# rust-cv/cv

Measured on NVIDIA H100. Metric: vSLAM frames/s (AKAZE+match+RANSAC, 1080p ~5k kp) at 1/2/4/8 H100, higher is better.
Workload: dtype f32+f64

## Files before the change

### cv_b200/csrc/arrsac_dev.cuh

```cuda
#pragma once

#define ARS_SORT_CAP 4096u
#define ARS_BOOK_NT 1024
#define ARS_BOOK_SMEM (14u * ARS_SORT_CAP)
#define ARS_QCAP (1u << 20)

struct ArrsacCtl {
    uint32_t n, init_n, Mv, npass;
    uint32_t Hn, cur, blk_lo, blk_hi;
    uint32_t acc_hi, n_new, worst, done;
    uint32_t found, iters, nraw, q_count;
    uint32_t q_count2, stat_lazy;
    uint32_t stat_units0, stat_units2;
    uint32_t stat_repairs, stat_pad;
    uint64_t rng_pos, gen_pos;
    cvb_rng gen;
    cvb_pose winner;
    uint32_t n_inliers, overflow;
    uint32_t stat_chunks, stat_pass;
    uint32_t stat_walk_us, stat_commit_us;
    uint32_t stat_perm_us, stat_turns;
};

struct ArrsacParams {
    uint32_t K, MM, kind;
    uint32_t H0, ib, bs, max_cand, G;
    uint32_t W0;
    uint32_t NW;
    uint32_t NMAX;
    uint32_t rows;
    uint32_t prefix, cmin;
    float lr_thr, eps0, delta0;
    double thr;
    int row0;
};

__device__ __forceinline__ unsigned long long ars_globaltimer() { unsigned long long t; asm volatile("mov.u64 %0, %%globaltimer;" : "=l"(t)); return t; }
__device__ __forceinline__ uint64_t ars_rotl64(uint64_t x, int k) { return (x << k) | (x >> (64 - k)); }
__device__ uint32_t ars_rng_next_u32(cvb_rng *r) {
    if (r->kind == 0) {
        uint64_t *s = r->s;
        const uint64_t result = ars_rotl64(s[0] + s[3], 23) + s[0];
        const uint64_t t = s[1] << 17;
        s[2] ^= s[0]; s[3] ^= s[1]; s[1] ^= s[2]; s[0] ^= s[3]; s[2] ^= t; s[3] = ars_rotl64(s[3], 45);
        return (uint32_t)(result >> 32);
    }
    unsigned __int128 state = (unsigned __int128)r->s[0] | ((unsigned __int128)r->s[1] << 64);
    const unsigned __int128 incr = (unsigned __int128)r->s[2] | ((unsigned __int128)r->s[3] << 64);
    const unsigned __int128 MUL = ((unsigned __int128)0x2360ED051FC65DA4ull << 64) | 0x4385DF649FCCF645ull;
    state = state * MUL + incr;
    r->s[0] = (uint64_t)state; r->s[1] = (uint64_t)(state >> 64);
    const uint32_t rot = (uint32_t)(state >> 122);
    const uint64_t xsl = (uint64_t)(state >> 64) ^ (uint64_t)state;
    return (uint32_t)((xsl >> rot) | (xsl << ((64 - rot) & 63)));
// ... 103 lines not shown
            }
            while (c < K) {
                const uint32_t s = ars_raw_at(ctl, raw, pos) % len;
                pos++;
                bool dup = false;
                for (uint32_t j = 0; j < c; j++) dup |= loc[j] == s;
                if (!dup) loc[c++] = s;
            }
            for (uint32_t k = 0; k < K; k++) out[(size_t)(h0 + f) * K + k] = loc[k];
            sh[0] = h0 + f + 1; *(uint64_t *)(sh + 2) = pos;
        } else if (f >= m && tid == 0) {
            sh[0] = h0 + m; *(uint64_t *)(sh + 2) = p0 + (uint64_t)m * K;
        }
        __syncthreads();
    }
    const uint32_t hdone = sh[0];
    __syncthreads();
    if (tid == 0) ctl->rng_pos = *(const uint64_t *)(sh + 2);
    __syncthreads();
    if (hdone < count) ars_sample_block(ctl, raw, len, K, count - hdone, out + (size_t)hdone * K, nullptr, win, sh);
}

__global__ void __launch_bounds__(ARS_BOOK_NT) k_ars_begin(ArrsacCtl *ctl, ArrsacParams P, const uint32_t *n_dev, uint32_t n_host,
                                                            const uint32_t *raw, uint32_t *samples0) {
    __shared__ uint32_t win[ARS_WIN];
    __shared__ __align__(8) uint32_t sh[4];
    const uint32_t n = min(n_dev ? *n_dev : n_host, P.NMAX);
    if (threadIdx.x == 0) {
        ctl->n = n;
        ctl->init_n = min(P.bs * P.ib, n);
        ctl->Mv = 0; ctl->npass = 0; ctl->Hn = 0; ctl->cur = 0; ctl->blk_lo = ctl->blk_hi = ctl->acc_hi = 0;
        ctl->n_new = 0; ctl->worst = 0; ctl->found = 0; ctl->iters = 0; ctl->n_inliers = 0; ctl->overflow = 0;
        ctl->stat_chunks = 0; ctl->stat_pass = 0; ctl->q_count = 0; ctl->q_count2 = 0; ctl->stat_lazy = 0; ctl->stat_units0 = 0; ctl->stat_units2 = 0; ctl->stat_repairs = 0; ctl->stat_pad = 0; ctl->stat_walk_us = 0; ctl->stat_commit_us = 0; ctl->stat_perm_us = 0; ctl->stat_turns = 0;
        ctl->done = (n < P.K || P.H0 == 0) ? 1u : 0u;
    }
    __syncthreads();
    if (n < P.K || P.H0 == 0) return;
    ars_sample_block_par(ctl, raw, n, P.K, P.H0, samples0, win, sh);
}

template <int KIND>
__global__ void __launch_bounds__(128) k_ars_estimate(const ArrsacCtl *ctl, int phase, uint32_t H_init, const double *__restrict__ a,
                                                      const double *__restrict__ b, const uint32_t *__restrict__ samples,
                                                      cvb_pose *poses, uint8_t *nposes, int row0) {
    if (ctl->done) return;
    const uint32_t H = phase == 0 ? H_init : ctl->n_new;
    const uint32_t h = blockIdx.x * blockDim.x + threadIdx.x;
    if (h >= H) return;
    if (KIND == 2) { nposes[h] = (uint8_t)five_point(a, b, samples + (size_t)h * 5, row0, poses + (size_t)h * 40); return; }
    cvb_pose out[4];
    const int n = KIND == 0 ? eight_point(a, b, samples + (size_t)h * 8, out) : p3p(a, b, samples + (size_t)h * 3, out);
    for (int k = 0; k < n; k++) poses[(size_t)h * 4 + k] = out[k];
    nposes[h] = (uint8_t)n;
}

template <int EIGHT_LANES, int MINB>
__global__ void __launch_bounds__(128, MINB) k_ars_estimate8(const ArrsacCtl *ctl, int phase, uint32_t H_init, const double *__restrict__ a,
                                                       const double *__restrict__ b, const uint32_t *__restrict__ samples,
                                                       cvb_pose *poses, uint8_t *nposes) {
    if (ctl->done) return;
    __shared__ double sh[(128 / EIGHT_LANES) * EIGHT_SH];
    const uint32_t H = phase == 0 ? H_init : ctl->n_new;
    const uint32_t g = threadIdx.x / EIGHT_LANES, lane = threadIdx.x % EIGHT_LANES;
    const uint32_t h = blockIdx.x * (128 / EIGHT_LANES) + g;
    if (h >= H) return;
    const unsigned mask = ((1u << EIGHT_LANES) - 1u) << ((threadIdx.x & 31) / EIGHT_LANES * EIGHT_LANES);
    cvb_pose out[4];
    const int n = eight_point_lanes<EIGHT_LANES>(a, b, samples + (size_t)h * 8, out, sh + g * EIGHT_SH, lane, mask);
    if (lane == 0) {
        for (int k = 0; k < n; k++) poses[(size_t)h * 4 + k] = out[k];
        nposes[h] = (uint8_t)n;
    }
}

__device__ __noinline__ bool ars_exact_c2c(const cvb_pose *Pz, const double *pa, const double *pb, double thr) {
    return residual_c2c(*Pz, pa, pb) < thr;
}

template <int RES>
__device__ __forceinline__ bool ars_inlier(const cvb_pose &Pz, const double *__restrict__ a, const double *__restrict__ b, uint32_t i,
                                           double thr) {
    if (RES == 1) return residual_w2c(Pz, a + 3 * (size_t)i, b + 4 * (size_t)i) < thr;
    const double *pa = a + 3 * (size_t)i, *pb = b + 3 * (size_t)i;
    int f = c2c_inlier_filter(Pz.r, Pz.t, pa, pb, thr);
    if (f < 0) f = ars_exact_c2c(&Pz, pa, pb, thr) ? 1 : 0;
    return f != 0;
}

__device__ __forceinline__ bool ars_ready(uint32_t word0, uint32_t init_n, uint32_t sample, const ArrsacParams &P) {
    if (sample < P.prefix) return true;
    const uint32_t c = min(32u, init_n);
    return (uint32_t)__popc(c < 32 ? (word0 & ((1u << c) - 1)) : word0) >= P.cmin;
}

template <int RES>
__global__ void __launch_bounds__(256, 2) k_ars_score(ArrsacCtl *ctl, uint2 *__restrict__ queue, ArrsacParams P, int phase, const double *__restrict__ a,
                                                   const double *__restrict__ b, const cvb_pose *__restrict__ poses0,
                                                   const uint8_t *__restrict__ nposes0, uint32_t *__restrict__ masks0,
                                                   const cvb_pose *__restrict__ tposes, uint32_t *__restrict__ tmasks,
                                                   const cvb_pose *__restrict__ newposes, const uint8_t *__restrict__ nposes_new,
                                                   uint32_t *__restrict__ newmask) {
    if (ctl->done) return;
    const unsigned full = 0xffffffffu;
    const uint32_t lane = threadIdx.x & 31;
    const uint32_t warp = (blockIdx.x * blockDim.x + threadIdx.x) >> 5, nwarps = (gridDim.x * blockDim.x) >> 5;
    if (phase == 0 || phase == 2) {
        const uint32_t init_n = ctl->init_n, W = (init_n + 31) >> 5;
        const uint32_t nmod = P.H0 * P.MM, npre = min(P.prefix, P.H0) * P.MM, W1 = W > 0 ? W - 1 : 0;
        const uint32_t units = phase == 0 ? nmod + npre * W1 : (nmod - npre) * W1;
        uint32_t *qc = phase == 0 ? &ctl->q_count : &ctl->q_count2;
        uint2 *q = phase == 0 ? queue : queue + ARS_QCAP;
        for (uint32_t u = warp; u < units; u += nwarps) {
            uint32_t m, w;
            if (phase == 0) { if (u < nmod) { m = u; w = 0; } else { m = (u - nmod) / W1; w = 1 + (u - nmod) % W1; } }
            else { m = npre + u / W1; w = 1 + u % W1; }
            if ((m % P.MM) >= nposes0[m / P.MM]) continue;
            if (phase == 2 && !ars_ready(masks0[(size_t)m * P.W0], init_n, m / P.MM, P)) continue;
            const uint32_t i = w * 32 + lane;
            bool bit = false;
            if (i < init_n) {
                if (RES == 1) bit = ars_inlier<RES>(poses0[m], a, b, i, P.thr);
                else {
                    const cvb_pose &Pz = poses0[m];
                    const int f = c2c_inlier_filter(Pz.r, Pz.t, a + 3 * (size_t)i, b + 3 * (size_t)i, P.thr);
                    if (f >= 0) bit = f != 0;
                    else {
                        const uint32_t slot = atomicAdd(qc, 1u);
                        if (slot < ARS_QCAP) q[slot] = make_uint2(m, i);
                        else bit = ars_exact_c2c(&Pz, a + 3 * (size_t)i, b + 3 * (size_t)i, P.thr);
                    }
                }
            }
            const unsigned bits = __ballot_sync(full, bit);
            if (lane == 0) { masks0[(size_t)m * P.W0 + w] = bits; atomicAdd(phase == 0 ? &ctl->stat_units0 : &ctl->stat_units2, 1u); }
        }
        return;
    }
    const uint32_t lo = ctl->blk_lo, hi = ctl->blk_hi, Hn = ctl->Hn, cur = ctl->cur;
    const uint32_t wlo = lo >> 5, nwb = hi > lo ? ((hi - 1) >> 5) - wlo + 1 : 0;
    const uint32_t kept_units = Hn * nwb;
    const uint32_t nnew = ctl->n_new * P.MM, nwn = (hi + 31) >> 5;
    const uint32_t units = kept_units + nnew * nwn;
    const cvb_pose *tp = tposes + (size_t)cur * P.rows;
    uint32_t *tm = tmasks + (size_t)cur * P.rows * P.NW;
    for (uint32_t u = warp; u < units; u += nwarps) {
        if (u < kept_units) {
            const uint32_t r = u / nwb, w = wlo + u % nwb;
            const uint32_t i = w * 32 + lane;
            const bool act = i >= lo && i < hi;
            bool bit = false;
            if (act) bit = ars_inlier<RES>(tp[r], a, b, i, P.thr);
            const unsigned bits = __ballot_sync(full, bit), range = __ballot_sync(full, act);
            if (lane == 0) { uint32_t *p = tm + (size_t)r * P.NW + w; *p = (*p & ~range) | bits; }
        } else {
            const uint32_t v = u - kept_units;
            const uint32_t j = v / nwn, w = v % nwn;
            if ((j % P.MM) >= nposes_new[j / P.MM]) continue;
            const uint32_t i = w * 32 + lane;
            bool bit = false;
            if (i < hi) bit = ars_inlier<RES>(newposes[j], a, b, i, P.thr);
            const unsigned bits = __ballot_sync(full, bit);
            if (lane == 0) newmask[(size_t)j * P.NW + w] = bits;
        }
    }
}

__global__ void __launch_bounds__(256) k_ars_resolve(const ArrsacCtl *ctl, const uint2 *__restrict__ queue, int stage, ArrsacParams P,
                                                     const double *__restrict__ a, const double *__restrict__ b,
                                                     const cvb_pose *__restrict__ poses0, uint32_t *__restrict__ masks0) {
    if (ctl->done) return;
    const uint32_t cnt = min(stage == 0 ? ctl->q_count : ctl->q_count2, ARS_QCAP);
    queue += stage == 0 ? 0 : ARS_QCAP;
    for (uint32_t e = blockIdx.x * blockDim.x + threadIdx.x; e < cnt; e += gridDim.x * blockDim.x) {
        const uint2 q = queue[e];
        if (residual_c2c(poses0[q.x], a + 3 * (size_t)q.y, b + 3 * (size_t)q.y) < P.thr)
            atomicOr(&masks0[(size_t)q.x * P.W0 + (q.y >> 5)], 1u << (q.y & 31));
    }
}

__device__ void ars_scan3(uint32_t &a, uint32_t &b, uint32_t &c, uint32_t *sm , uint32_t *tot ) {
    const unsigned full = 0xffffffffu;
    const uint32_t lane = threadIdx.x & 31, wid = threadIdx.x >> 5;
    for (int o = 1; o < 32; o <<= 1) {
        const uint32_t x = __shfl_up_sync(full, a, o), y = __shfl_up_sync(full, b, o), z = __shfl_up_sync(full, c, o);
        if ((int)lane >= o) { a += x; b += y; c += z; }
    }
    __syncthreads();
    if (lane == 31) { sm[wid] = a; sm[32 + wid] = b; sm[64 + wid] = c; }
    __syncthreads();
    if (wid == 0) {
        uint32_t x = sm[lane], y = sm[32 + lane], z = sm[64 + lane];
        for (int o = 1; o < 32; o <<= 1) {
            const uint32_t p = __shfl_up_sync(full, x, o), q = __shfl_up_sync(full, y, o), r = __shfl_up_sync(full, z, o);
            if ((int)lane >= o) { x += p; y += q; z += r; }
        }
        sm[lane] = x; sm[32 + lane] = y; sm[64 + lane] = z;
        if (lane == 31) { tot[0] = x; tot[1] = y; tot[2] = z; }
    }
    __syncthreads();
    if (wid > 0) { a += sm[wid - 1]; b += sm[32 + wid - 1]; c += sm[64 + wid - 1]; }
}

__device__ uint32_t ars_block_min(uint32_t v, uint32_t *sm ) {
    const unsigned full = 0xffffffffu;
    for (int o = 16; o; o >>= 1) v = min(v, __shfl_xor_sync(full, v, o));
    __syncthreads();
    if ((threadIdx.x & 31) == 0) sm[threadIdx.x >> 5] = v;
    __syncthreads();
    uint32_t r = sm[threadIdx.x & 31];
// ... 355 lines not shown
        const uint32_t id = vm[p];
        const double *src = (const double *)(poses0 + id);
        double *dst = (double *)(tposes + r);
        if (lane < 12) dst[lane] = src[lane];
        if (lane == 0) tinl[r] = 0xfffffu - (uint32_t)(kx >> 32);
        for (uint32_t w = lane; w < P.NW; w += 32) tmasks[(size_t)r * P.NW + w] = w < P.W0 ? masks0[(size_t)id * P.W0 + w] : 0u;
    }
    __syncthreads();
    if (tid == 0) {
        const uint32_t n = ctl->n;
        ctl->Hn = Hn; ctl->cur = 0; ctl->stat_pass = npass;
        ctl->acc_hi = init_n; ctl->blk_lo = init_n; ctl->blk_hi = min(init_n + P.bs, n);
        ctl->n_new = 0; ctl->worst = 0;
        if (!(init_n < n && Hn > 1)) {
            ctl->done = 1; ctl->found = Hn >= 1 ? 1 : 0;
            if (Hn >= 1) ctl->winner = tposes[0];
        }
    }
}

__global__ void __launch_bounds__(ARS_BOOK_NT) k_ars_book(ArrsacCtl *ctl, ArrsacParams P, const uint32_t *__restrict__ raw,
                                                           cvb_pose *tposes, uint32_t *tinl, uint32_t *tmasks,
                                                           const cvb_pose *__restrict__ newposes, const uint8_t *__restrict__ nposes_new,
                                                           const uint32_t *__restrict__ newmask, uint32_t *__restrict__ pool,
                                                           uint32_t *__restrict__ samples_new, unsigned long long loop_cond) {
    if (ctl->done) { if (loop_cond && threadIdx.x == 0) cudaGraphSetConditional(loop_cond, 0); return; }
    __shared__ __align__(8) uint32_t sm[96];
    __shared__ uint32_t tot[3];
    extern __shared__ __align__(16) unsigned char ars_dyn[];
    uint64_t *keys = (uint64_t *)ars_dyn;
    uint32_t *e_inl = (uint32_t *)(ars_dyn + 8 * ARS_SORT_CAP);
    uint16_t *e_src = (uint16_t *)(ars_dyn + 12 * ARS_SORT_CAP);
    const uint32_t tid = threadIdx.x, NT = blockDim.x;
    const uint32_t cur = ctl->cur, Hk = ctl->Hn, n = ctl->n;
    const uint32_t acc_hi = ctl->acc_hi, lo = ctl->blk_lo, hi = ctl->blk_hi, worst = ctl->worst;
    const uint32_t nnew = ctl->n_new * P.MM;
    const cvb_pose *tp = tposes + (size_t)cur * P.rows;
    const uint32_t *ti = tinl + (size_t)cur * P.rows;
    const uint32_t *tm = tmasks + (size_t)cur * P.rows * P.NW;
    for (uint32_t r = tid; r < Hk; r += NT) { e_inl[r] = ti[r]; e_src[r] = (uint16_t)r; keys[r] = ars_key(ti[r], r, r); }
    uint32_t total = Hk;
    for (uint32_t j0 = 0; j0 < nnew; j0 += NT) {
        const uint32_t j = j0 + tid;
        uint32_t inl = 0;
        bool acc = false;
        if (j < nnew && (j % P.MM) < nposes_new[j / P.MM]) {
            inl = ars_popc_range(newmask + (size_t)j * P.NW, 0, acc_hi);
            acc = inl > worst;
        }
        uint32_t x = acc ? 1 : 0, y = 0, z = 0;
        ars_scan3(x, y, z, sm, tot);
        if (acc) {
            const uint32_t p = total + x - 1;
            if (p < ARS_SORT_CAP) { e_inl[p] = inl; e_src[p] = (uint16_t)(P.rows + j); keys[p] = ars_key(inl, p, p); }
        }
        total += tot[0];
        __syncthreads();
    }
    uint32_t P2 = ars_pow2(max(total, 2u));
    for (uint32_t i = total + tid; i < P2; i += NT) keys[i] = ~0ull;
    ars_bitonic(keys, P2);
    const uint32_t Hn1 = min(total, P.max_cand);
    if (!(lo < n && Hn1 > 1)) {
        if (tid == 0) {
            ctl->done = 1; ctl->found = Hn1 >= 1 ? 1 : 0;
            if (Hn1 >= 1) {
// ... 100 lines not shown
```

### cv_b200/csrc/c2c_filter.cuh

```cuda
#pragma once
#include <math.h>

#if defined(__CUDACC__)
#define C2C_HD __host__ __device__ __forceinline__
#else
#define C2C_HD static inline
#endif
#if defined(__CUDA_ARCH__)
#define C2C_FMA(a, b, c) fma((a), (b), (c))
#define C2C_RSQRT(a) rsqrt(a)
#else
#define C2C_FMA(a, b, c) ((a) * (b) + (c))
#define C2C_RSQRT(a) (1.0 / sqrt(a))
#endif

C2C_HD int c2c_ldl4(const double *m, double s, double *d, double *l, double *inv) {
    const double tiny = 1e-11;
    const double m00 = m[0] - s, m11 = m[5] - s, m22 = m[10] - s, m33 = m[15] - s;
    const double m10 = m[4], m20 = m[8], m30 = m[12], m21 = m[9], m31 = m[13], m32 = m[14];
    int neg = 0;
    d[0] = m00;
    if (!(fabs(d[0]) > tiny)) return -1;
    neg += d[0] < 0.0;
    const double i0 = 1.0 / d[0];
// ... 48 lines not shown
        const double c0 = C2C_FMA(t[1], ra2, -(t[2] * ra1)), c1 = C2C_FMA(t[2], ra0, -(t[0] * ra2)), c2 = C2C_FMA(t[0], ra1, -(t[1] * ra0));
        const double e = C2C_FMA(b[2], c2, C2C_FMA(b[1], c1, b[0] * c0));
        if (e * e > 8.5 * (tt - 1.0) * thr + 1e-28) return 0;
        if (thr <= 1e-4) {
            const double tb = C2C_FMA(t[2], b[2], C2C_FMA(t[1], b[1], t[0] * b[0])), ub = C2C_FMA(ra2, b[2], C2C_FMA(ra1, b[1], ra0 * b[0])),
                         tu = C2C_FMA(t[2], ra2, C2C_FMA(t[1], ra1, t[0] * ra0));
            const double c1 = C2C_FMA(-ub, tu, tb), c2 = C2C_FMA(ub, tb, -tu);
            const double lim2 = 100.0 * (tt - 1.0) * thr;
            if ((c1 < 0.0 && c1 * c1 > lim2) || (c2 < 0.0 && c2 * c2 > lim2)) return 0;
        }
    }
    double D[16];
    {
        double Ta[3][3];
        for (int c = 0; c < 3; c++)
            for (int r = 0; r < 3; r++) Ta[r][c] = C2C_FMA(-a[r], a[c], r == c ? 1.0 : 0.0);
        double Tb[3][4];
        for (int c = 0; c < 4; c++) {
            const double m0 = c < 3 ? R[c] : t[0], m1 = c < 3 ? R[3 + c] : t[1], m2 = c < 3 ? R[6 + c] : t[2];
            const double btm = C2C_FMA(b[2], m2, C2C_FMA(b[1], m1, b[0] * m0));
            Tb[0][c] = C2C_FMA(-b[0], btm, m0); Tb[1][c] = C2C_FMA(-b[1], btm, m1); Tb[2][c] = C2C_FMA(-b[2], btm, m2);
        }
        for (int i = 0; i < 4; i++)
            for (int j = 0; j <= i; j++) {
                double v = C2C_FMA(Tb[2][i], Tb[2][j], C2C_FMA(Tb[1][i], Tb[1][j], Tb[0][i] * Tb[0][j]));
                if (i < 3) v = C2C_FMA(Ta[2][i], Ta[2][j], C2C_FMA(Ta[1][i], Ta[1][j], C2C_FMA(Ta[0][i], Ta[0][j], v)));
                D[i * 4 + j] = v; D[j * 4 + i] = v;
            }
    }
    double d[4], l[6], id[4], dh[4], lh[6], ih[4];
    const int c_lo = c2c_ldl4(D, s_lo, d, l, id);
    if (c_lo == 0) return 0;
    if (c_lo != 1) return -1;
    if (c2c_ldl4(D, s_hi, dh, lh, ih) != 1) return -1;
    id[3] = 1.0 / d[3];
    double x[4] = {0.5, 0.5, 0.5, 0.5};
    c2c_ldl4_solve(id, l, x);
    c2c_ldl4_solve(id, l, x);
    c2c_ldl4_solve(id, l, x);
    c2c_ldl4_solve(id, l, x);
    c2c_normalise4(x);
    double y[4], yy = 0.0;
    int certified = 0;
    for (int it = 0; it < 4; it++) {
        y[0] = x[0]; y[1] = x[1]; y[2] = x[2]; y[3] = x[3];
        c2c_ldl4_solve(id, l, y);
        const double xy = c2c_dot4(x, y);
        yy = c2c_dot4(y, y);
        double r2 = 0.0;
        for (int k = 0; k < 4; k++) { const double r = C2C_FMA(-xy, x[k], y[k]); r2 = C2C_FMA(r, r, r2); }
        if (r2 <= 1e-22 * yy) { certified = 1; break; }
        const double in = C2C_RSQRT(yy);
        for (int k = 0; k < 4; k++) x[k] = y[k] * in;
    }
    if (!certified) return -1;
    double p[4] = {y[0], y[1], y[2], y[3]};
    if (signbit(p[3])) { p[0] = -p[0]; p[1] = -p[1]; p[2] = -p[2]; p[3] = -p[3]; }
    const double pp = p[0] * p[0] + p[1] * p[1] + p[2] * p[2];
    if (!(pp > 1e-18 * yy)) return -1;
    const double ipn = C2C_RSQRT(pp);
    p[0] *= ipn; p[1] *= ipn; p[2] *= ipn; p[3] *= ipn;
    double q[3];
    for (int r = 0; r < 3; r++) q[r] = R[3 * r] * p[0] + R[3 * r + 1] * p[1] + R[3 * r + 2] * p[2] + t[r] * p[3];
    const double qq = q[0] * q[0] + q[1] * q[1] + q[2] * q[2];
    if (!(qq > 1e-18)) return -1;
    const double res = 0.5 * (1.0 - (a[0] * p[0] + a[1] * p[1] + a[2] * p[2]) + 1.0 - (b[0] * q[0] + b[1] * q[1] + b[2] * q[2]) * C2C_RSQRT(qq));
    if (!isfinite(res)) return -1;
    if (fabs(res - thr) <= 1e-11 + 1e-4 * thr) return -1;
    return res < thr ? 1 : 0;
}
```

### cv_b200/csrc/geom.cu

```cuda
#include <math.h>
#include <stdio.h>
#include <stdlib.h>
#include <string.h>
#include <algorithm>
#include <vector>
#include "common.cuh"
#include "../../include/cvb200_tri.h"
#include "c2c_filter.cuh"
#include "pinhole.cuh"

namespace {

__device__ __forceinline__ void jacobi_cs(double app, double aqq, double apq, double &c, double &s) {
    const double theta = __ddiv_rn(__dsub_rn(aqq, app), __dmul_rn(2.0, apq));
    const double t = __ddiv_rn(theta >= 0.0 ? 1.0 : -1.0, __dadd_rn(fabs(theta), __dsqrt_rn(__dadd_rn(__dmul_rn(theta, theta), 1.0))));
    c = __ddiv_rn(1.0, __dsqrt_rn(__dadd_rn(__dmul_rn(t, t), 1.0)));
    s = __dmul_rn(t, c);
}
__device__ __forceinline__ void jacobi_rot(double &x, double &y, double c, double s) {
    const double a = x, b = y;
    x = __dsub_rn(__dmul_rn(c, a), __dmul_rn(s, b));
    y = __dadd_rn(__dmul_rn(s, a), __dmul_rn(c, b));
}

// ... 1247 lines not shown
}

struct DevBuf {
    void *p = nullptr;
    size_t bytes = 0;
    int ensure(cvb_ctx *ctx, size_t need) {
        if (need <= bytes && p) return 0;
        if (p) { cvb_wait(ctx, ctx->stream); cudaFree(p); p = nullptr; bytes = 0; }
        size_t n = std::max<size_t>(need, 256);
        cudaError_t e = cudaMalloc(&p, n);
        if (e != cudaSuccess) return cvb_set_error(ctx, CVB_ENOMEM, "cudaMalloc(%zu): %s", n, cudaGetErrorString(e));
        bytes = n;
        return 0;
    }
};

}

struct ArsWorkspace {
    DevBuf ctl, raw, samples0, poses0, nposes0, masks0, vm, pass_id, pass_inl, tposes, tinl, tmasks, newposes, nposes_new, newmask,
        pool, samples_new, res, queue;
    uint32_t *h_raw = nullptr;
    size_t h_raw_cap = 0;
    unsigned char *h_res = nullptr;
    cudaEvent_t up_done = nullptr;
    std::vector<cvb_rng> snaps;
    cvb_rng rng0;
    uint32_t nraw = 0;
    bool pending = false;
    struct GraphKey {
        ArrsacParams P; int kind, row0; const void *a, *b, *n_dev; uint32_t n_host, nmax, cap, nb; const void *model, *inl, *ninl, *found;
        const void *ws[21];
    };
    struct GraphEntry { GraphKey key; cudaGraphExec_t exec; uint64_t launches; bool loop; };
    bool last_loop = false;
    std::vector<GraphEntry> graphs;
    std::vector<GraphKey> seen;
    int use_graph = -1;
    int use_while = -1;
    cudaStream_t body_stream = nullptr;
};
struct GeomWorkspace {
    DevBuf a, b, samples, poses, nposes, out, masks, offsets, ok;
    ArsWorkspace *ars = nullptr;
};
void geom_workspace_free(GeomWorkspace *g) {
    if (!g) return;
    DevBuf *bufs[] = {&g->a, &g->b, &g->samples, &g->poses, &g->nposes, &g->out, &g->masks, &g->offsets, &g->ok};
    for (DevBuf *d : bufs) if (d->p) cudaFree(d->p);
    if (g->ars) {
        ArsWorkspace *w = g->ars;
        DevBuf *ab[] = {&w->ctl, &w->raw, &w->samples0, &w->poses0, &w->nposes0, &w->masks0, &w->vm, &w->pass_id, &w->pass_inl, &w->tposes,
                        &w->tinl, &w->tmasks, &w->newposes, &w->nposes_new, &w->newmask, &w->pool, &w->samples_new, &w->res, &w->queue};
        for (DevBuf *d : ab) if (d->p) cudaFree(d->p);
        if (w->h_raw) cudaFreeHost(w->h_raw);
        if (w->h_res) cudaFreeHost(w->h_res);
        if (w->up_done) cudaEventDestroy(w->up_done);
        if (w->body_stream) cudaStreamDestroy(w->body_stream);
        for (auto &ge : w->graphs) cudaGraphExecDestroy(ge.exec);
        delete w;
    }
    delete g;
}

namespace {

inline uint32_t kind_K(int kind) { return kind == 0 ? 8u : (kind == 1 ? 3u : 5u); }
inline uint32_t kind_M(int kind) { return kind == 2 ? 40u : 4u; }
// ... 266 lines not shown
        if (w->h_raw) { cvb_wait(ctx, ctx->stream); cudaFreeHost(w->h_raw); w->h_raw = nullptr; w->h_raw_cap = 0; }
        if (cudaHostAlloc((void **)&w->h_raw, stage_bytes, cudaHostAllocDefault) != cudaSuccess) return cvb_set_error(ctx, CVB_ENOMEM, "page-locked staging");
        w->h_raw_cap = stage_bytes;
    }
    if (!w->h_res && cudaHostAlloc((void **)&w->h_res, sizeof(ArrsacCtl) + sizeof(cvb_pose) + 64, cudaHostAllocDefault) != cudaSuccess)
        return cvb_set_error(ctx, CVB_ENOMEM, "page-locked staging");
    if (!w->up_done) CVB_CUDA(ctx, cudaEventCreateWithFlags(&w->up_done, cudaEventDisableTiming | cudaEventBlockingSync));
    else CVB_CUDA(ctx, cudaEventSynchronize(w->up_done));
    {
        cvb_rng g = *rng;
        w->rng0 = g;
        w->snaps.clear();
        uint32_t *raw = (uint32_t *)((unsigned char *)w->h_raw + hdr);
        for (uint32_t i = 0; i < nraw; i++) {
            if (i % ARS_SNAP == 0) w->snaps.push_back(g);
            raw[i] = cvb_rng_next_u32(&g);
        }
        ArrsacCtl *h = (ArrsacCtl *)w->h_raw;
        memset(h, 0, sizeof(*h));
        h->nraw = nraw; h->gen = g; h->gen_pos = nraw; h->rng_pos = 0;
        w->nraw = nraw;
    }
    cudaStream_t st = ctx->stream;
    static bool attr_set = false;
    if (!attr_set) {
        cudaFuncSetAttribute(k_ars_book, cudaFuncAttributeMaxDynamicSharedMemorySize, (int)ARS_BOOK_SMEM);
        cudaFuncSetAttribute(k_ars_sprt<0>, cudaFuncAttributeMaxDynamicSharedMemorySize, 64 * 1024);
        cudaFuncSetAttribute(k_ars_sprt<1>, cudaFuncAttributeMaxDynamicSharedMemorySize, 64 * 1024);
        cudaFuncSetAttribute(k_ars_score<0>, cudaFuncAttributeMaxDynamicSharedMemorySize, 200 * 1024);
        cudaFuncSetAttribute(k_ars_score<1>, cudaFuncAttributeMaxDynamicSharedMemorySize, 200 * 1024);
        attr_set = true;
    }
    bool capturing = false, while_loop = false;
    auto enqueue = [&]() -> int {
        CVB_CUDA(ctx, cudaMemcpyAsync(w->ctl.p, w->h_raw, sizeof(ArrsacCtl), cudaMemcpyHostToDevice, st));
        CVB_CUDA(ctx, cudaMemcpyAsync(w->raw.p, (unsigned char *)w->h_raw + hdr, sizeof(uint32_t) * (size_t)nraw, cudaMemcpyHostToDevice, st));
        if (!capturing) CVB_CUDA(ctx, cudaEventRecord(w->up_done, st));
        ArrsacCtl *ctl = (ArrsacCtl *)w->ctl.p;
        const uint32_t *raw = (const uint32_t *)w->raw.p;
        const int res = kind_res(kind);
        {
            CVB_PROF(ctx, "k_ars_begin", 0);
            k_ars_begin<<<1, ARS_BOOK_NT, 0, st>>>(ctl, P, n_dev, n_host, raw, (uint32_t *)w->samples0.p);
            CVB_LAUNCH_CHECK(ctx);
        }
        auto estimate = [&](int phase, uint32_t H, const uint32_t *samples, cvb_pose *poses, uint8_t *nposes) -> int {
            if (H == 0) return 0;
            CVB_PROF(ctx, phase == 0 ? "k_ars_estimate_init" : "k_ars_estimate_block", 0);
            if (kind == 0 && phase == 0) k_ars_estimate8<4, 5><<<cdiv(H, 128 / 4), 128, 0, st>>>(ctl, phase, H, a_dev, b_dev, samples, poses, nposes);
            else if (kind == 0) k_ars_estimate8<16, 5><<<cdiv(H, 128 / 16), 128, 0, st>>>(ctl, phase, H, a_dev, b_dev, samples, poses, nposes);
            else if (kind == 1) k_ars_estimate<1><<<cdiv(H, 128), 128, 0, st>>>(ctl, phase, H, a_dev, b_dev, samples, poses, nposes, row0);
            else k_ars_estimate<2><<<cdiv(H, 128), 128, 0, st>>>(ctl, phase, H, a_dev, b_dev, samples, poses, nposes, row0);
            CVB_LAUNCH_CHECK(ctx);
            return 0;
        };
    const uint32_t sgrid_full = (uint32_t)ctx->num_sms * 4;
        uint32_t sgrid_block = 48;
        if (const char *e = getenv("CVB_ARS_SGRID")) sgrid_block = (uint32_t)std::max(1, atoi(e));
        size_t score_smem = 0;
        if (const char *e = getenv("CVB_ARS_SCORE_SMEM")) score_smem = (size_t)std::max(0, atoi(e));
        auto score = [&](int phase) -> int {
            const uint32_t sgrid = phase == 1 ? sgrid_block : sgrid_full;
            CVB_PROF(ctx, phase == 1 ? "k_ars_score_block" : "k_ars_score_init", 0);
            if (res == 0)
                k_ars_score<0><<<sgrid, 256, score_smem, st>>>(ctl, (uint2 *)w->queue.p, P, phase, a_dev, b_dev, (const cvb_pose *)w->poses0.p, (const uint8_t *)w->nposes0.p,
                                                      (uint32_t *)w->masks0.p, (const cvb_pose *)w->tposes.p, (uint32_t *)w->tmasks.p,
// ... 11 lines not shown
            k_ars_resolve<<<sgrid_full, 256, 0, st>>>(ctl, (const uint2 *)w->queue.p, stage, P, a_dev, b_dev, (const cvb_pose *)w->poses0.p, (uint32_t *)w->masks0.p);
            CVB_LAUNCH_CHECK(ctx);
            return 0;
        };
        if ((rc = score(0))) return rc;
        if (res == 0 && (rc = resolve(0))) return rc;
        if (P.prefix < P.H0 && P.W0 > 1) {
            if ((rc = score(2))) return rc;
            if (res == 0 && (rc = resolve(1))) return rc;
        }
        {
            CVB_PROF(ctx, "k_ars_sprt", 0);
            if (res == 0)
                k_ars_sprt<0><<<1, ARS_BOOK_NT, 8 * ARS_SORT_CAP, st>>>(ctl, P, a_dev, b_dev, (const cvb_pose *)w->poses0.p, (const uint8_t *)w->nposes0.p, (uint32_t *)w->masks0.p,
                                                        (uint32_t *)w->vm.p, (uint32_t *)w->pass_id.p, (uint32_t *)w->pass_inl.p, (cvb_pose *)w->tposes.p,
                                                        (uint32_t *)w->tinl.p, (uint32_t *)w->tmasks.p);
            else
                k_ars_sprt<1><<<1, ARS_BOOK_NT, 8 * ARS_SORT_CAP, st>>>(ctl, P, a_dev, b_dev, (const cvb_pose *)w->poses0.p, (const uint8_t *)w->nposes0.p, (uint32_t *)w->masks0.p,
                                                        (uint32_t *)w->vm.p, (uint32_t *)w->pass_id.p, (uint32_t *)w->pass_inl.p, (cvb_pose *)w->tposes.p,
                                                        (uint32_t *)w->tinl.p, (uint32_t *)w->tmasks.p);
            CVB_LAUNCH_CHECK(ctx);
        }
        const uint32_t n_bound = n_dev ? P.NMAX : std::min(n_host, P.NMAX);
        const uint32_t init_n = std::min(P.bs * P.ib, n_bound);
        const uint32_t nb = n_bound > init_n ? cdiv(n_bound - init_n, P.bs) : 0;
        auto book = [&](unsigned long long cond) -> int {
            CVB_PROF(ctx, "k_ars_book", 0);
            k_ars_book<<<1, ARS_BOOK_NT, ARS_BOOK_SMEM, st>>>(ctl, P, raw, (cvb_pose *)w->tposes.p, (uint32_t *)w->tinl.p, (uint32_t *)w->tmasks.p,
                                                              (const cvb_pose *)w->newposes.p, (const uint8_t *)w->nposes_new.p,
                                                              (const uint32_t *)w->newmask.p, (uint32_t *)w->pool.p, (uint32_t *)w->samples_new.p, cond);
            CVB_LAUNCH_CHECK(ctx);
            return 0;
        };
        if (capturing && while_loop) {
            cudaStreamCaptureStatus cs;
            cudaGraph_t g = nullptr;
            const cudaGraphNode_t *deps = nullptr;
            size_t ndeps = 0;
            CVB_CUDA(ctx, cudaStreamGetCaptureInfo(st, &cs, nullptr, &g, &deps, &ndeps));
            cudaGraphConditionalHandle cond;
            CVB_CUDA(ctx, cudaGraphConditionalHandleCreate(&cond, g, 1, cudaGraphCondAssignDefault));
            cudaGraphNodeParams np = {cudaGraphNodeTypeConditional};
            np.conditional.handle = cond;
            np.conditional.type = cudaGraphCondTypeWhile;
            np.conditional.size = 1;
            cudaGraphNode_t node;
            CVB_CUDA(ctx, cudaGraphAddNode(&node, g, deps, ndeps, &np));
            cudaGraph_t body = np.conditional.phGraph_out[0];
            const cudaStream_t outer = st;
            CVB_CUDA(ctx, cudaStreamBeginCaptureToGraph(w->body_stream, body, nullptr, nullptr, 0, cudaStreamCaptureModeThreadLocal));
            st = w->body_stream;
            rc = score(1);
            if (!rc) rc = book(cond);
            if (!rc && nb && P.G) rc = estimate(1, P.G, (const uint32_t *)w->samples_new.p, (cvb_pose *)w->newposes.p, (uint8_t *)w->nposes_new.p);
            cudaGraph_t same_body = nullptr;
            const cudaError_t be = cudaStreamEndCapture(st, &same_body);
            st = outer;
            if (rc) return rc;
            CVB_CUDA(ctx, be);
            CVB_CUDA(ctx, cudaStreamUpdateCaptureDependencies(st, &node, 1, cudaStreamSetCaptureDependencies));
        } else
        for (uint32_t it = 0; it <= nb; it++) {
            if ((rc = score(1))) return rc;
            if ((rc = book(0))) return rc;
            if (it < nb && P.G)
                if ((rc = estimate(1, P.G, (const uint32_t *)w->samples_new.p, (cvb_pose *)w->newposes.p, (uint8_t *)w->nposes_new.p))) return rc;
        }
        {
            CVB_PROF(ctx, "k_ars_final", 0);
            if (res == 0) k_ars_final<0><<<1, ARS_BOOK_NT, 0, st>>>(ctl, P, a_dev, b_dev, model_dev, inl_dev, cap, ninl_dev, found_dev);
            else k_ars_final<1><<<1, ARS_BOOK_NT, 0, st>>>(ctl, P, a_dev, b_dev, model_dev, inl_dev, cap, ninl_dev, found_dev);
            CVB_LAUNCH_CHECK(ctx);
        }
        CVB_CUDA(ctx, cudaMemcpyAsync(w->h_res, w->ctl.p, sizeof(ArrsacCtl), cudaMemcpyDeviceToHost, st));
        return 0;
    };
    if (w->use_graph < 0) {
        const char *e1 = getenv("CVB_NO_GRAPH"), *e2 = getenv("CVB_ARS_NO_GRAPH");
        w->use_graph = ((e1 && e1[0] == '1') || (e2 && e2[0] == '1')) ? 0 : 1;
    }
    if (!w->use_graph || ctx->prof) {
        if ((rc = enqueue())) return rc;
        w->pending = true;
        return 0;
    }
    ArsWorkspace::GraphKey key;
    memset(&key, 0, sizeof(key));
    key.P = P; key.kind = kind; key.row0 = row0; key.a = a_dev; key.b = b_dev; key.n_dev = n_dev; key.n_host = n_host; key.nmax = nmax; key.cap = cap;
    key.model = model_dev; key.inl = inl_dev; key.ninl = ninl_dev; key.found = found_dev;
    {
        const DevBuf *bufs[] = {&w->ctl, &w->raw, &w->samples0, &w->poses0, &w->nposes0, &w->masks0, &w->vm, &w->pass_id, &w->pass_inl, &w->tposes,
                                &w->tinl, &w->tmasks, &w->newposes, &w->nposes_new, &w->newmask, &w->pool, &w->samples_new, &w->queue};
        int i = 0;
        for (const DevBuf *d : bufs) key.ws[i++] = d->p;
        key.ws[i++] = w->h_raw; key.ws[i++] = w->h_res; key.ws[i++] = (const void *)(uintptr_t)nraw;
    }
    auto same = [](const ArsWorkspace::GraphKey &x, const ArsWorkspace::GraphKey &y) { return memcmp(&x, &y, sizeof(x)) == 0; };
    for (auto &ge : w->graphs)
        if (same(ge.key, key)) {
            CVB_CUDA(ctx, cudaGraphLaunch(ge.exec, st));
            CVB_CUDA(ctx, cudaEventRecord(w->up_done, st));
            ctx->launches += ge.launches;
            w->last_loop = ge.loop;
            w->pending = true;
            return 0;
        }
    bool seen = false;
    for (auto &k : w->seen) seen = seen || same(k, key);
    if (!seen) {
        if (w->seen.size() >= 64) w->seen.erase(w->seen.begin());
        w->seen.push_back(key);
        if ((rc = enqueue())) return rc;
        w->pending = true;
        return 0;
    }
    const uint64_t l0 = ctx->launches;
    if (w->use_while < 0) {
        const char *e = getenv("CVB_ARS_WHILE");
        w->use_while = (e && e[0] == '0') ? 0 : 1;
    }
    if (w->use_while && !w->body_stream && cudaStreamCreateWithFlags(&w->body_stream, cudaStreamNonBlocking) != cudaSuccess) {
        cudaGetLastError();
        w->use_while = 0;
    }
    cudaGraphExec_t exec = nullptr;
    cudaError_t ce = cudaSuccess;
    for (int attempt = 0; attempt < 2 && !exec; attempt++) {
        ctx->launches = l0;
        capturing = true;
        while_loop = w->use_while != 0;
        CVB_CUDA(ctx, cudaStreamBeginCapture(st, cudaStreamCaptureModeThreadLocal));
        rc = enqueue();
        cudaGraph_t graph = nullptr;
        ce = cudaStreamEndCapture(st, &graph);
        capturing = false;
        if (!rc && ce == cudaSuccess && graph) ce = cudaGraphInstantiate(&exec, graph, 0);
        if (graph) cudaGraphDestroy(graph);
        if (exec || !while_loop) break;
        cudaGetLastError();
        w->use_while = 0;
        exec = nullptr;
    }
    if (rc) return rc;
    if (ce != cudaSuccess || !exec) {
        cudaGetLastError();
        w->use_graph = 0;
        ctx->launches = l0;
        if ((rc = enqueue())) return rc;
        w->pending = true;
        return 0;
    }
    if (w->graphs.size() >= 16) { cudaGraphExecDestroy(w->graphs.front().exec); w->graphs.erase(w->graphs.begin()); }
    w->graphs.push_back({key, exec, ctx->launches - l0, while_loop});
    w->last_loop = while_loop;
    CVB_CUDA(ctx, cudaGraphLaunch(exec, st));
    CVB_CUDA(ctx, cudaEventRecord(w->up_done, st));
    w->pending = true;
    return 0;
}

int arrsac_commit_rng(cvb_ctx *ctx, cvb_rng *rng, ArrsacCtl *stats_out = nullptr) {
    ArsWorkspace *w = arsws(ctx);
    if (!w->pending) return cvb_set_error(ctx, CVB_EINVAL, "no device ARRSAC run to commit");
    const ArrsacCtl *h = (const ArrsacCtl *)w->h_res;
    if (stats_out) *stats_out = *h;
    if (w->last_loop) ctx->launches += 3ull * h->iters;
    w->last_loop = false;
    w->pending = false;
    if (!rng) return 0;
    const uint64_t used = h->rng_pos;
    if (used >= w->nraw) {
        if (h->gen_pos != std::max<uint64_t>(used, w->nraw)) return cvb_set_error(ctx, CVB_ECUDA, "generator position mismatch");
        *rng = h->gen;
        return 0;
    }
    cvb_rng g = w->snaps[used / ARS_SNAP];
    for (uint64_t i = used / ARS_SNAP * ARS_SNAP; i < used; i++) cvb_rng_next_u32(&g);
    *rng = g;
    return 0;
}

int arrsac_host(cvb_ctx *ctx, const cvb_arrsac_cfg *cfg, int kind, const double *a, const double *b, uint32_t n, cvb_rng *rng,
                cvb_pose *model_out, uint32_t *inliers_out, uint32_t cap, uint32_t *n_inliers, int32_t *found, int row0 = 5) {
    *found = 0;
    if (n_inliers) *n_inliers = 0;
    if (n < kind_K(kind) || cfg->initialization_hypotheses == 0) return 0;
    CVB_CUDA(ctx, cudaSetDevice(ctx->device));
    int rc = upload_data(ctx, kind, a, b, n);
    if (rc) return rc;
    GeomWorkspace *g = gws(ctx);
    ArsWorkspace *w = arsws(ctx);
    const size_t res_bytes = sizeof(cvb_pose) + 16 + sizeof(uint32_t) * (size_t)n;
    if ((rc = w->res.ensure(ctx, res_bytes))) return rc;
    unsigned char *rd = (unsigned char *)w->res.p;
    cvb_pose *model_dev = (cvb_pose *)rd;
    uint32_t *ninl_dev = (uint32_t *)(rd + sizeof(cvb_pose));
    int32_t *found_dev = (int32_t *)(rd + sizeof(cvb_pose) + 4);
    uint32_t *inl_dev = (uint32_t *)(rd + sizeof(cvb_pose) + 16);
    if ((rc = arrsac_run_dev(ctx, cfg, kind, (const double *)g->a.p, (const double *)g->b.p, nullptr, n, n, rng, model_dev, inl_dev, n, ninl_dev,
                             found_dev, row0))) return rc;
// ... 284 lines not shown
    if (!kp_a_dev || !kp_b_dev || !pairs_dev || !n_pairs_dev || !intrinsics || !a_out_dev || !b_out_dev) return cvb_set_error(ctx, CVB_EINVAL, "null argument");
    if (cap == 0) return 0;
    CVB_CUDA(ctx, cudaSetDevice(ctx->device));
    CVB_PROF(ctx, "k_pair_bearings", 0);
    k_pair_bearings<<<cdiv(cap, 256), 256, 0, ctx->stream>>>(kp_a_dev, kp_b_dev, pairs_dev, n_pairs_dev, cap, *intrinsics, a_out_dev, b_out_dev);
    CVB_LAUNCH_CHECK(ctx);
    return 0;
}

static int arrsac_dev_entry(cvb_ctx *ctx, const cvb_arrsac_cfg *cfg, int kind, const double *a_dev, const double *b_dev, const uint32_t *n_dev,
                            uint32_t n_max, const cvb_rng *rng, cvb_pose *model_out_dev, uint32_t *inliers_out_dev, uint32_t cap,
                            uint32_t *n_inliers_dev, int32_t *found_dev) {
    if (!ctx) return CVB_EINVAL;
    if (!cfg || !rng || !a_dev || !b_dev || !n_dev || !model_out_dev || !n_inliers_dev || !found_dev) return cvb_set_error(ctx, CVB_EINVAL, "null argument");
    CVB_CUDA(ctx, cudaSetDevice(ctx->device));
    return arrsac_run_dev(ctx, cfg, kind, a_dev, b_dev, n_dev, 0, n_max, rng, model_out_dev, inliers_out_dev, cap, n_inliers_dev, found_dev, 5);
}
int cvb_arrsac_eight_point_dev(cvb_ctx *ctx, const cvb_arrsac_cfg *cfg, const double *a_dev, const double *b_dev, const uint32_t *n_dev,
                               uint32_t n_max, const cvb_rng *rng, cvb_pose *model_out_dev, uint32_t *inliers_out_dev, uint32_t cap,
                               uint32_t *n_inliers_dev, int32_t *found_dev) {
    return arrsac_dev_entry(ctx, cfg, 0, a_dev, b_dev, n_dev, n_max, rng, model_out_dev, inliers_out_dev, cap, n_inliers_dev, found_dev);
}
int cvb_arrsac_p3p_dev(cvb_ctx *ctx, const cvb_arrsac_cfg *cfg, const double *bearings_dev, const double *world_dev, const uint32_t *n_dev,
                       uint32_t n_max, const cvb_rng *rng, cvb_pose *model_out_dev, uint32_t *inliers_out_dev, uint32_t cap,
                       uint32_t *n_inliers_dev, int32_t *found_dev) {
    return arrsac_dev_entry(ctx, cfg, 1, bearings_dev, world_dev, n_dev, n_max, rng, model_out_dev, inliers_out_dev, cap, n_inliers_dev, found_dev);
}
int cvb_arrsac_commit_rng(cvb_ctx *ctx, cvb_rng *rng, uint32_t *stats_out) {
    if (!ctx) return CVB_EINVAL;
    CVB_CUDA(ctx, cvb_wait(ctx, ctx->stream));
    ArrsacCtl h;
    int rc = arrsac_commit_rng(ctx, rng, &h);
    if (rc) return rc;
    if (getenv("CVB_ARS_DEBUG"))
        fprintf(stderr, "[arrsac] n %u models %u pass %u chunks %u turns %u repairs %u lazy %u | sprt us: order %u walk %u commit %u | block iterations %u\n", h.n, h.Mv, h.npass,
                h.stat_chunks, h.stat_turns, h.stat_repairs, h.stat_lazy, h.stat_perm_us, h.stat_walk_us, h.stat_commit_us, h.iters);
    if (stats_out) {
        stats_out[0] = h.n; stats_out[1] = h.Mv; stats_out[2] = h.npass; stats_out[3] = h.stat_chunks; stats_out[4] = h.iters;
        stats_out[5] = (uint32_t)h.rng_pos; stats_out[6] = h.n_inliers; stats_out[7] = h.found;
        stats_out[8] = h.stat_units0; stats_out[9] = h.stat_units2; stats_out[10] = h.q_count + h.q_count2; stats_out[11] = h.stat_lazy;
        stats_out[12] = h.stat_repairs; stats_out[13] = h.stat_pad ; stats_out[14] = h.stat_walk_us; stats_out[15] = h.stat_commit_us;
    }
    return 0;
}

int cvb_single_view_optimize_l2(cvb_ctx *ctx, const cvb_pose *poses, uint32_t B, double optimization_rate, uint32_t iterations,
                                const double *bearings, const double *world, const uint32_t *offsets, cvb_pose *poses_out,
                                uint32_t *updates_out) {
    if (!ctx) return CVB_EINVAL;
    if (B == 0) return 0;
    if (!poses || !offsets || !poses_out) return cvb_set_error(ctx, CVB_EINVAL, "null argument");
    for (uint32_t b = 0; b < B; b++)
        if (offsets[b + 1] < offsets[b]) return cvb_set_error(ctx, CVB_EINVAL, "offsets must be non-decreasing");
    const uint32_t n = offsets[B];
    if (n && (!bearings || !world)) return cvb_set_error(ctx, CVB_EINVAL, "null argument");
    CVB_CUDA(ctx, cudaSetDevice(ctx->device));
    GeomWorkspace *g = gws(ctx);
    int rc;
    if ((rc = upload(ctx, g->poses, poses, sizeof(cvb_pose) * (size_t)B))) return rc;
    if ((rc = upload(ctx, g->a, bearings, sizeof(double) * 3 * (size_t)n))) return rc;
    if ((rc = upload(ctx, g->b, world, sizeof(double) * 4 * (size_t)n))) return rc;
    if ((rc = upload(ctx, g->offsets, offsets, sizeof(uint32_t) * ((size_t)B + 1)))) return rc;
    if ((rc = g->out.ensure(ctx, sizeof(cvb_pose) * (size_t)B))) return rc;
    if ((rc = g->ok.ensure(ctx, sizeof(uint32_t) * (size_t)B))) return rc;
    {
        CVB_PROF(ctx, "k_single_view_opt", 0.0);
        k_single_view_opt<<<B, OPT_NT, 0, ctx->stream>>>((const cvb_pose *)g->poses.p, (const double *)g->a.p, (const double *)g->b.p,
                                                         (const uint32_t *)g->offsets.p, optimization_rate, iterations, (cvb_pose *)g->out.p,
                                                         (uint32_t *)g->ok.p);
// ... 99 lines not shown
```

Before: 1483.

## Defer undecided block-phase inlier checks to a resolve kernel and strengthen filter

The block-phase scoring used to run the exact c2c residual inline for every pair the cheap filter could not decide, which makes warps diverge. Those pairs are now pushed onto a queue and settled by a new k_ars_resolve_block kernel inside the while-loop body, matching what the initial phases already do. The c2c filter also retries its high-shift LDL with smaller shifts and allows up to 12 power iterations instead of 4, so fewer pairs reach the exact path. The cost is one extra kernel launch per loop iteration, atomics on the queue counter, and more filter work for hard cases; launch accounting and the debug print are moved to match.

```diff
diff --git a/cv_b200/csrc/arrsac_dev.cuh b/cv_b200/csrc/arrsac_dev.cuh
--- a/cv_b200/csrc/arrsac_dev.cuh
+++ b/cv_b200/csrc/arrsac_dev.cuh
@@ -20,6 +20,7 @@
     uint32_t stat_chunks, stat_pass;
     uint32_t stat_walk_us, stat_commit_us;
     uint32_t stat_perm_us, stat_turns;
+    uint32_t q_blk, stat_qblk;
 };
 
 struct ArrsacParams {
@@ -189,6 +190,7 @@
         ctl->Mv = 0; ctl->npass = 0; ctl->Hn = 0; ctl->cur = 0; ctl->blk_lo = ctl->blk_hi = ctl->acc_hi = 0;
         ctl->n_new = 0; ctl->worst = 0; ctl->found = 0; ctl->iters = 0; ctl->n_inliers = 0; ctl->overflow = 0;
         ctl->stat_chunks = 0; ctl->stat_pass = 0; ctl->q_count = 0; ctl->q_count2 = 0; ctl->stat_lazy = 0; ctl->stat_units0 = 0; ctl->stat_units2 = 0; ctl->stat_repairs = 0; ctl->stat_pad = 0; ctl->stat_walk_us = 0; ctl->stat_commit_us = 0; ctl->stat_perm_us = 0; ctl->stat_turns = 0;
+        ctl->q_blk = 0; ctl->stat_qblk = 0;
         ctl->done = (n < P.K || P.H0 == 0) ? 1u : 0u;
     }
     __syncthreads();
@@ -242,6 +244,18 @@
     int f = c2c_inlier_filter(Pz.r, Pz.t, pa, pb, thr);
     if (f < 0) f = ars_exact_c2c(&Pz, pa, pb, thr) ? 1 : 0;
     return f != 0;
+}
+
+template <int RES>
+__device__ __forceinline__ bool ars_inlier_queued(const cvb_pose &Pz, const double *__restrict__ a, const double *__restrict__ b, uint32_t i,
+                                                  double thr, uint32_t *qc, uint2 *q, uint32_t src) {
+    if (RES == 1) return ars_inlier<RES>(Pz, a, b, i, thr);
+    const double *pa = a + 3 * (size_t)i, *pb = b + 3 * (size_t)i;
+    const int f = c2c_inlier_filter(Pz.r, Pz.t, pa, pb, thr);
+    if (f >= 0) return f != 0;
+    const uint32_t slot = atomicAdd(qc, 1u);
+    if (slot < ARS_QCAP) { q[slot] = make_uint2(src, i); return false; }
+    return ars_exact_c2c(&Pz, pa, pb, thr);
 }
 
 __device__ __forceinline__ bool ars_ready(uint32_t word0, uint32_t init_n, uint32_t sample, const ArrsacParams &P) {
@@ -275,19 +289,7 @@
             if (phase == 2 && !ars_ready(masks0[(size_t)m * P.W0], init_n, m / P.MM, P)) continue;
             const uint32_t i = w * 32 + lane;
             bool bit = false;
-            if (i < init_n) {
-                if (RES == 1) bit = ars_inlier<RES>(poses0[m], a, b, i, P.thr);
-                else {
-                    const cvb_pose &Pz = poses0[m];
-                    const int f = c2c_inlier_filter(Pz.r, Pz.t, a + 3 * (size_t)i, b + 3 * (size_t)i, P.thr);
-                    if (f >= 0) bit = f != 0;
-                    else {
-                        const uint32_t slot = atomicAdd(qc, 1u);
-                        if (slot < ARS_QCAP) q[slot] = make_uint2(m, i);
-                        else bit = ars_exact_c2c(&Pz, a + 3 * (size_t)i, b + 3 * (size_t)i, P.thr);
-                    }
-                }
-            }
+            if (i < init_n) bit = ars_inlier_queued<RES>(poses0[m], a, b, i, P.thr, qc, q, m);
             const unsigned bits = __ballot_sync(full, bit);
             if (lane == 0) { masks0[(size_t)m * P.W0 + w] = bits; atomicAdd(phase == 0 ? &ctl->stat_units0 : &ctl->stat_units2, 1u); }
         }
@@ -306,7 +308,7 @@
             const uint32_t i = w * 32 + lane;
             const bool act = i >= lo && i < hi;
             bool bit = false;
-            if (act) bit = ars_inlier<RES>(tp[r], a, b, i, P.thr);
+            if (act) bit = ars_inlier_queued<RES>(tp[r], a, b, i, P.thr, &ctl->q_blk, queue, r);
             const unsigned bits = __ballot_sync(full, bit), range = __ballot_sync(full, act);
             if (lane == 0) { uint32_t *p = tm + (size_t)r * P.NW + w; *p = (*p & ~range) | bits; }
         } else {
@@ -315,7 +317,7 @@
             if ((j % P.MM) >= nposes_new[j / P.MM]) continue;
             const uint32_t i = w * 32 + lane;
             bool bit = false;
-            if (i < hi) bit = ars_inlier<RES>(newposes[j], a, b, i, P.thr);
+            if (i < hi) bit = ars_inlier_queued<RES>(newposes[j], a, b, i, P.thr, &ctl->q_blk, queue, P.rows + j);
             const unsigned bits = __ballot_sync(full, bit);
             if (lane == 0) newmask[(size_t)j * P.NW + w] = bits;
         }
@@ -332,6 +334,21 @@
         const uint2 q = queue[e];
         if (residual_c2c(poses0[q.x], a + 3 * (size_t)q.y, b + 3 * (size_t)q.y) < P.thr)
             atomicOr(&masks0[(size_t)q.x * P.W0 + (q.y >> 5)], 1u << (q.y & 31));
+    }
+}
+
+__global__ void __launch_bounds__(64) k_ars_resolve_block(const ArrsacCtl *ctl, const uint2 *__restrict__ queue, ArrsacParams P,
+                                                          const double *__restrict__ a, const double *__restrict__ b,
+                                                          const cvb_pose *__restrict__ tposes, uint32_t *__restrict__ tmasks,
+                                                          const cvb_pose *__restrict__ newposes, uint32_t *__restrict__ newmask) {
+    if (ctl->done) return;
+    const uint32_t cnt = min(ctl->q_blk, ARS_QCAP), cur = ctl->cur;
+    for (uint32_t e = blockIdx.x * blockDim.x + threadIdx.x; e < cnt; e += gridDim.x * blockDim.x) {
+        const uint2 q = queue[e];
+        const bool kept = q.x < P.rows;
+        const size_t row = kept ? (size_t)cur * P.rows + q.x : (size_t)(q.x - P.rows);
+        if (residual_c2c(kept ? tposes[row] : newposes[row], a + 3 * (size_t)q.y, b + 3 * (size_t)q.y) < P.thr)
+            atomicOr(&(kept ? tmasks : newmask)[row * P.NW + (q.y >> 5)], 1u << (q.y & 31));
     }
 }
 
@@ -753,6 +770,7 @@
     uint32_t *e_inl = (uint32_t *)(ars_dyn + 8 * ARS_SORT_CAP);
     uint16_t *e_src = (uint16_t *)(ars_dyn + 12 * ARS_SORT_CAP);
     const uint32_t tid = threadIdx.x, NT = blockDim.x;
+    if (tid == 0) { ctl->stat_qblk += ctl->q_blk; ctl->q_blk = 0; }
     const uint32_t cur = ctl->cur, Hk = ctl->Hn, n = ctl->n;
     const uint32_t acc_hi = ctl->acc_hi, lo = ctl->blk_lo, hi = ctl->blk_hi, worst = ctl->worst;
     const uint32_t nnew = ctl->n_new * P.MM;
diff --git a/cv_b200/csrc/c2c_filter.cuh b/cv_b200/csrc/c2c_filter.cuh
--- a/cv_b200/csrc/c2c_filter.cuh
+++ b/cv_b200/csrc/c2c_filter.cuh
@@ -104,7 +104,10 @@
     const int c_lo = c2c_ldl4(D, s_lo, d, l, id);
     if (c_lo == 0) return 0;
     if (c_lo != 1) return -1;
-    if (c2c_ldl4(D, s_hi, dh, lh, ih) != 1) return -1;
+    for (double s = s_hi; c2c_ldl4(D, s, dh, lh, ih) != 1;) {
+        s *= 0.125;
+        if (!(s >= 16.0 * s_lo)) return -1;
+    }
     id[3] = 1.0 / d[3];
     double x[4] = {0.5, 0.5, 0.5, 0.5};
     c2c_ldl4_solve(id, l, x);
@@ -114,7 +117,7 @@
     c2c_normalise4(x);
     double y[4], yy = 0.0;
     int certified = 0;
-    for (int it = 0; it < 4; it++) {
+    for (int it = 0; it < 12; it++) {
         y[0] = x[0]; y[1] = x[1]; y[2] = x[2]; y[3] = x[3];
         c2c_ldl4_solve(id, l, y);
         const double xy = c2c_dot4(x, y);
diff --git a/cv_b200/csrc/geom.cu b/cv_b200/csrc/geom.cu
--- a/cv_b200/csrc/geom.cu
+++ b/cv_b200/csrc/geom.cu
@@ -1303,8 +1303,8 @@
         ArrsacParams P; int kind, row0; const void *a, *b, *n_dev; uint32_t n_host, nmax, cap, nb; const void *model, *inl, *ninl, *found;
         const void *ws[21];
     };
-    struct GraphEntry { GraphKey key; cudaGraphExec_t exec; uint64_t launches; bool loop; };
-    bool last_loop = false;
+    struct GraphEntry { GraphKey key; cudaGraphExec_t exec; uint64_t launches; uint32_t body; };
+    uint32_t last_body = 0;
     std::vector<GraphEntry> graphs;
     std::vector<GraphKey> seen;
     int use_graph = -1;
@@ -1637,6 +1637,7 @@
         attr_set = true;
     }
     bool capturing = false, while_loop = false;
+    uint32_t body_launches = 0;
     auto enqueue = [&]() -> int {
         CVB_CUDA(ctx, cudaMemcpyAsync(w->ctl.p, w->h_raw, sizeof(ArrsacCtl), cudaMemcpyHostToDevice, st));
         CVB_CUDA(ctx, cudaMemcpyAsync(w->raw.p, (unsigned char *)w->h_raw + hdr, sizeof(uint32_t) * (size_t)nraw, cudaMemcpyHostToDevice, st));
@@ -1714,6 +1715,16 @@
             CVB_LAUNCH_CHECK(ctx);
             return 0;
         };
+        auto score_block = [&](unsigned long long cond) -> int {
+            if ((rc = score(1))) return rc;
+            if (res == 0) {
+                CVB_PROF(ctx, "k_ars_resolve_block", 0);
+                k_ars_resolve_block<<<sgrid_full, 64, 0, st>>>(ctl, (const uint2 *)w->queue.p, P, a_dev, b_dev, (const cvb_pose *)w->tposes.p,
+                                                               (uint32_t *)w->tmasks.p, (const cvb_pose *)w->newposes.p, (uint32_t *)w->newmask.p);
+                CVB_LAUNCH_CHECK(ctx);
+            }
+            return book(cond);
+        };
         if (capturing && while_loop) {
             cudaStreamCaptureStatus cs;
             cudaGraph_t g = nullptr;
@@ -1732,9 +1743,10 @@
             const cudaStream_t outer = st;
             CVB_CUDA(ctx, cudaStreamBeginCaptureToGraph(w->body_stream, body, nullptr, nullptr, 0, cudaStreamCaptureModeThreadLocal));
             st = w->body_stream;
-            rc = score(1);
-            if (!rc) rc = book(cond);
+            const uint64_t b0 = ctx->launches;
+            rc = score_block(cond);
             if (!rc && nb && P.G) rc = estimate(1, P.G, (const uint32_t *)w->samples_new.p, (cvb_pose *)w->newposes.p, (uint8_t *)w->nposes_new.p);
+            body_launches = (uint32_t)(ctx->launches - b0);
             cudaGraph_t same_body = nullptr;
             const cudaError_t be = cudaStreamEndCapture(st, &same_body);
             st = outer;
@@ -1743,8 +1755,7 @@
             CVB_CUDA(ctx, cudaStreamUpdateCaptureDependencies(st, &node, 1, cudaStreamSetCaptureDependencies));
         } else
         for (uint32_t it = 0; it <= nb; it++) {
-            if ((rc = score(1))) return rc;
-            if ((rc = book(0))) return rc;
+            if ((rc = score_block(0))) return rc;
             if (it < nb && P.G)
                 if ((rc = estimate(1, P.G, (const uint32_t *)w->samples_new.p, (cvb_pose *)w->newposes.p, (uint8_t *)w->nposes_new.p))) return rc;
         }
@@ -1783,7 +1794,7 @@
             CVB_CUDA(ctx, cudaGraphLaunch(ge.exec, st));
             CVB_CUDA(ctx, cudaEventRecord(w->up_done, st));
             ctx->launches += ge.launches;
-            w->last_loop = ge.loop;
+            w->last_body = ge.body;
             w->pending = true;
             return 0;
         }
@@ -1833,8 +1844,8 @@
         return 0;
     }
     if (w->graphs.size() >= 16) { cudaGraphExecDestroy(w->graphs.front().exec); w->graphs.erase(w->graphs.begin()); }
-    w->graphs.push_back({key, exec, ctx->launches - l0, while_loop});
-    w->last_loop = while_loop;
+    w->graphs.push_back({key, exec, ctx->launches - l0, while_loop ? body_launches : 0u});
+    w->last_body = while_loop ? body_launches : 0u;
     CVB_CUDA(ctx, cudaGraphLaunch(exec, st));
     CVB_CUDA(ctx, cudaEventRecord(w->up_done, st));
     w->pending = true;
@@ -1846,8 +1857,12 @@
     if (!w->pending) return cvb_set_error(ctx, CVB_EINVAL, "no device ARRSAC run to commit");
     const ArrsacCtl *h = (const ArrsacCtl *)w->h_res;
     if (stats_out) *stats_out = *h;
-    if (w->last_loop) ctx->launches += 3ull * h->iters;
-    w->last_loop = false;
+    if (getenv("CVB_ARS_DEBUG"))
+        fprintf(stderr, "[arrsac] n %u models %u pass %u chunks %u turns %u repairs %u lazy %u | sprt us: order %u walk %u commit %u | block iterations %u"
+                " | undecided predicates queued: initial %u block %u\n", h->n, h->Mv, h->npass, h->stat_chunks, h->stat_turns, h->stat_repairs,
+                h->stat_lazy, h->stat_perm_us, h->stat_walk_us, h->stat_commit_us, h->iters, h->q_count + h->q_count2, h->stat_qblk);
+    ctx->launches += (uint64_t)w->last_body * h->iters;
+    w->last_body = 0;
     w->pending = false;
     if (!rng) return 0;
     const uint64_t used = h->rng_pos;
@@ -2198,9 +2213,6 @@
     ArrsacCtl h;
     int rc = arrsac_commit_rng(ctx, rng, &h);
     if (rc) return rc;
-    if (getenv("CVB_ARS_DEBUG"))
-        fprintf(stderr, "[arrsac] n %u models %u pass %u chunks %u turns %u repairs %u lazy %u | sprt us: order %u walk %u commit %u | block iterations %u\n", h.n, h.Mv, h.npass,
-                h.stat_chunks, h.stat_turns, h.stat_repairs, h.stat_lazy, h.stat_perm_us, h.stat_walk_us, h.stat_commit_us, h.iters);
     if (stats_out) {
         stats_out[0] = h.n; stats_out[1] = h.Mv; stats_out[2] = h.npass; stats_out[3] = h.stat_chunks; stats_out[4] = h.iters;
         stats_out[5] = (uint32_t)h.rng_pos; stats_out[6] = h.n_inliers; stats_out[7] = h.found;
```

Result: faster. 1553, median of 6 (+4.7%).
